# wengroup/matten

Hardware: NVIDIA B200
Metric: crystals/sec (inference fwd) (higher is better)
Workload: dtype f32

## Files before the change

matten_b200/csrc/conv_fwd_tc.cu:

```cuda
#include <stdlib.h>

#include <cub/device/device_scan.cuh>

#include "conv_fwd_tc.cuh"

namespace mt {

constexpr size_t kTcSmemLimit = (size_t)227 * 1024 - 1024;

static int tc_pick_ne(const mt_conv_tc_part& part, int y_lmax) {
  static const int cand[] = {256, 128, 80, 64, 48, 32};
  const int y_pad = sh_pad_len(y_lmax);
  for (int ne : cand) {
    if (2 * part.num_tiles * ne > 512) continue;
    const TcSmemLayout L = tc_smem_layout(part.a_rows, part.x_cols, y_pad, part.num_bi, ne);
    if (L.total <= kTcSmemLimit) return ne;
  }
  return 0;
}

static bool tc_plan_qualifies(const mt_conv_plan* plan) {
  if (plan->tc_num_parts <= 0 || plan->tc_num_parts > MT_TC_MAX_PARTS) return false;
  if (plan->tc_y_lmax < 0 || plan->tc_y_lmax > MT_LMAX) return false;
  if (plan->mlp_num_layers > 3) return false;
// ... 78 lines not shown
  const TcLayout L = tc_layout(y_lmax, N, E);
  MT_REQUIRE(layout && layout_bytes >= L.total && (reinterpret_cast<uintptr_t>(layout) & 255) == 0,
             "conv layout: buffer of mt_conv_layout_bytes() bytes, 256-byte aligned, required");
  MT_REQUIRE(rowptr && (E == 0 || (sh && perm && src_sorted)), "null pointer");
  return tc_prepare_layout(L, reinterpret_cast<uintptr_t>(layout), y_lmax, static_cast<const float*>(sh), rowptr, perm,
                           src_sorted, N, as_stream(stream));
}

size_t conv_fwd_tc_workspace_bytes(const mt_conv_plan* plan, int64_t N, int64_t E) {
  if (!tc_plan_qualifies(plan) || N <= 0) return 0;
  return tc_workspace_bytes(tc_layout(plan->tc_y_lmax, N, E));
}

static long long* g_tc_dbg = nullptr;
void conv_fwd_tc_set_debug(void* p) { g_tc_dbg = static_cast<long long*>(p); }

typedef CUresult (*EncodeTiledFn)(CUtensorMap*, CUtensorMapDataType, cuuint32_t, void*, const cuuint64_t*, const cuuint64_t*,
                                  const cuuint32_t*, const cuuint32_t*, CUtensorMapInterleave, CUtensorMapSwizzle,
                                  CUtensorMapL2promotion, CUtensorMapFloatOOBfill);

static EncodeTiledFn encode_tiled_fn() {
  static EncodeTiledFn fn = nullptr;
  static bool tried = false;
  if (!tried) {
    void* p = nullptr;
    cudaDriverEntryPointQueryResult q;
    if (cudaGetDriverEntryPoint("cuTensorMapEncodeTiled", &p, cudaEnableDefault, &q) == cudaSuccess &&
        q == cudaDriverEntryPointSuccess)
      fn = reinterpret_cast<EncodeTiledFn>(p);
    tried = true;
  }
  return fn;
}

int conv_fwd_tc_try(const mt_conv_plan* plan, const void* x, const void* sh, const void* emb,
                    const void* const* mlp_weights, const int32_t* rowptr, const int32_t* perm,
                    const int32_t* src_sorted, double avg, const void* num_neigh, void* out, void* workspace,
                    size_t workspace_bytes, const void* layout, int64_t N, int64_t E, cudaStream_t st, int* used) {
  *used = 0;
  if (!tc_plan_qualifies(plan)) return MT_OK;
  if (E + 3 * N >= (int64_t)2147483647 || N >= (int64_t)2147483647) return MT_OK;
  const TcLayout L = tc_layout(plan->tc_y_lmax, N, E);
  if (workspace == nullptr || workspace_bytes < tc_workspace_bytes(L)) return MT_OK;
  if ((reinterpret_cast<uintptr_t>(x) & 15) != 0) return MT_OK;
  EncodeTiledFn encode = encode_tiled_fn();
  if (encode == nullptr) return set_error(MT_ECUDA, "cuTensorMapEncodeTiled is not available from this driver");
  ConvTcParams p;
  memset(&p, 0, sizeof(p));
  p.x_dim = plan->x_dim;
  p.y_dim = plan->y_dim;
  p.y_lmax = plan->tc_y_lmax;
  p.out_dim = plan->out_dim;
  p.nl = plan->mlp_num_layers;
  for (int i = 0; i <= p.nl; ++i) p.sizes[i] = plan->mlp_sizes[i];
  for (int i = 0; i < p.nl; ++i) p.w[i] = static_cast<const float*>(mlp_weights[i]);
  p.act = plan->mlp_act;
  p.act_cst = (float)plan->mlp_act_cst;
  p.emb = static_cast<const float*>(emb);
  p.rowptr = rowptr;
  p.perm = perm;
  p.src = src_sorted;
  p.avg = (float)avg;
  p.num_neigh = static_cast<const float*>(num_neigh);
  p.out = static_cast<float*>(out);
  p.N = N;
  p.E = E;
  p.num_parts = plan->tc_num_parts;
  p.dbg = g_tc_dbg;
  {
    const uintptr_t base = (reinterpret_cast<uintptr_t>(workspace) + 255) & ~(uintptr_t)255;
    if (layout == nullptr) {
      const int rc = tc_prepare_layout(L, base, plan->tc_y_lmax, static_cast<const float*>(sh), rowptr, perm, src_sorted,
                                       N, st);
      if (rc != MT_OK) return rc;
      layout = reinterpret_cast<const void*>(base);
    }
    const uintptr_t lb = reinterpret_cast<uintptr_t>(layout);
    p.rowptr_pad = reinterpret_cast<int32_t*>(lb + L.rowptr_pad) + (N + 1);
    p.orig_pad = reinterpret_cast<int32_t*>(lb + L.orig_pad);
    p.src_pad = reinterpret_cast<int32_t*>(lb + L.src_pad);
    p.ypairs = reinterpret_cast<float*>(lb + L.ypairs);
    p.hplanes = reinterpret_cast<__nv_bfloat16*>(base + L.total);
    p.cols_max = L.cols_max;
    const bool fast = p.nl == 3 && p.sizes[0] <= 8 && p.sizes[1] == kTcK && p.sizes[2] == kTcK && p.act == MT_ACT_SILU;
    int64_t g = ceil_div<int64_t>(L.cols_max, fast ? 256 : 64);
    if (g > (int64_t)kNumSMs * 8) g = (int64_t)kNumSMs * 8;
    if (g < 1) g = 1;
    if (fast) tc_edge_hidden_fast_kernel<<<(unsigned)g, 256, 0, st>>>(p);
    else tc_edge_hidden_kernel<<<(unsigned)g, kHidThreads, 0, st>>>(p);
    MT_LAUNCH_OK();
  }
  int64_t grid = kNumSMs;
  if (grid > N * p.num_parts) grid = N * p.num_parts;
  if (grid < p.num_parts) grid = p.num_parts;
  double cost_sum = 0;
  for (int i = 0; i < p.num_parts; ++i) cost_sum += plan->tc_parts[i].cost > 0 ? plan->tc_parts[i].cost : 1;
  int assigned = 0;
  int lmax = 0;
  TcMaps maps;
  memset(&maps, 0, sizeof(maps));
  size_t smem_max = 0;
  for (int i = 0; i < p.num_parts; ++i) {
    const mt_conv_tc_part& pt = plan->tc_parts[i];
    TcPartParams& q = p.part[i];
    q.num_tiles = pt.num_tiles;
    q.a_rows = pt.a_rows;
    q.num_bi = pt.num_bi;
    q.x_lo = pt.x_lo;
    q.x_cols = pt.x_cols;
    q.ne = tc_pick_ne(pt, plan->tc_y_lmax);
    for (int k = 0; k < 4; ++k) q.q_count[k] = pt.q_count[k];
    q.row_wcol = pt.row_wcol;
    q.bi_hdr = pt.bi_hdr;
    q.bi_lane = pt.bi_lane;
    q.q_list = pt.q_list;
    const double c = pt.cost > 0 ? pt.cost : 1;
    int n = (i + 1 == p.num_parts) ? (int)grid - assigned : (int)((double)grid * c / cost_sum + 0.5);
    const int left = p.num_parts - 1 - i;
    if (n > (int)grid - assigned - left) n = (int)grid - assigned - left;
    if (n < 1) n = 1;
    if (n > N && N > 0) n = (int)N;
    q.cta_first = assigned;
    q.cta_count = n;
    assigned += n;
    if (pt.lmax > lmax) lmax = pt.lmax;
    const TcSmemLayout L = tc_smem_layout(q.a_rows, q.x_cols, sh_pad_len(p.y_lmax), q.num_bi, q.ne);
    if (L.total > smem_max) smem_max = L.total;
    cuuint64_t dims[2] = {(cuuint64_t)plan->x_dim, (cuuint64_t)(N > 0 ? N : 1)};
    cuuint64_t strides[1] = {(cuuint64_t)plan->x_dim * 4};
    cuuint32_t box[2] = {(cuuint32_t)q.x_cols, 1};
    cuuint32_t estr[2] = {1, 1};
    const CUresult r = encode(&maps.m[i], CU_TENSOR_MAP_DATA_TYPE_FLOAT32, 2, const_cast<void*>(x), dims, strides, box, estr,
                              CU_TENSOR_MAP_INTERLEAVE_NONE, CU_TENSOR_MAP_SWIZZLE_NONE, CU_TENSOR_MAP_L2_PROMOTION_NONE,
                              CU_TENSOR_MAP_FLOAT_OOB_FILL_NONE);
    if (r != CUDA_SUCCESS) return set_error(MT_ECUDA, "cuTensorMapEncodeTiled failed (%d)", (int)r);
    cuuint64_t hdims[3] = {16, (cuuint64_t)p.cols_max, 12};
    cuuint64_t hstrides[2] = {16, (cuuint64_t)p.cols_max * 16};
    cuuint32_t hbox[3] = {16, (cuuint32_t)q.ne, 12};
    cuuint32_t hestr[3] = {1, 1, 1};
    const CUresult rh = encode(&maps.h[i], CU_TENSOR_MAP_DATA_TYPE_UINT8, 3, p.hplanes, hdims, hstrides, hbox, hestr,
                               CU_TENSOR_MAP_INTERLEAVE_NONE, CU_TENSOR_MAP_SWIZZLE_NONE, CU_TENSOR_MAP_L2_PROMOTION_NONE,
                               CU_TENSOR_MAP_FLOAT_OOB_FILL_NONE);
    if (rh != CUDA_SUCCESS) return set_error(MT_ECUDA, "cuTensorMapEncodeTiled (h planes) failed (%d)", (int)rh);
  }
  grid = assigned;
  static thread_local size_t configured[2] = {0, 0};
  const int vi = lmax <= 2 ? 0 : 1;
  if (smem_max > configured[vi]) {
    if (vi == 0)
      MT_CUDA_OK(cudaFuncSetAttribute(conv_fwd_tc_kernel<2>, cudaFuncAttributeMaxDynamicSharedMemorySize, (int)kTcSmemLimit));
    else
      MT_CUDA_OK(cudaFuncSetAttribute(conv_fwd_tc_kernel<4>, cudaFuncAttributeMaxDynamicSharedMemorySize, (int)kTcSmemLimit));
    configured[vi] = kTcSmemLimit;
  }
  if (vi == 0) conv_fwd_tc_kernel<2><<<(unsigned)grid, kTcThreads, smem_max, st>>>(p, maps);
  else conv_fwd_tc_kernel<4><<<(unsigned)grid, kTcThreads, smem_max, st>>>(p, maps);
  MT_LAUNCH_OK();
  *used = 1;
  return MT_OK;
}

}
```

matten_b200/csrc/conv_fwd_tc.cuh:

```cuda
#pragma once
#include <cuda.h>
#include <cuda_bf16.h>

#include "common.cuh"
#include "generated/cg_bundles.cuh"

namespace mt {

constexpr int kTcK = 32;
constexpr int kTcProducerWarps = 4;
constexpr int kTcConsumerWarps = 16;
constexpr int kTcThreads = 32 * (kTcProducerWarps + kTcConsumerWarps);
constexpr int kTcMaxTiles = 4;
constexpr int kTcMaxBI = 64;
constexpr int kTcMaxNodes = 32;
constexpr int kTcMaxParts = 4;

__host__ __device__ constexpr int tc_chunk_cols(int MT) { return MT <= 1 ? 256 : (MT == 2 ? 128 : (MT == 3 ? 80 : 64)); }

struct TcPartParams {
  int num_tiles;
  int a_rows;
  int num_bi;
  int x_lo, x_cols;
// ... 81 lines not shown
}
__device__ __forceinline__ void fence_barrier_init() { asm volatile("fence.mbarrier_init.release.cluster;" ::: "memory"); }
__device__ __forceinline__ void fence_proxy_async() { asm volatile("fence.proxy.async.shared::cta;" ::: "memory"); }
__device__ __forceinline__ void tc_fence_before() { asm volatile("tcgen05.fence::before_thread_sync;" ::: "memory"); }
__device__ __forceinline__ void tc_fence_after() { asm volatile("tcgen05.fence::after_thread_sync;" ::: "memory"); }
__device__ __forceinline__ void tmem_alloc(uint32_t* dst_smem, uint32_t ncols) {
  asm volatile("tcgen05.alloc.cta_group::1.sync.aligned.shared::cta.b32 [%0], %1;" ::"r"(smem_u32(dst_smem)), "r"(ncols)
               : "memory");
  asm volatile("tcgen05.relinquish_alloc_permit.cta_group::1.sync.aligned;" ::: "memory");
}
__device__ __forceinline__ void tmem_dealloc(uint32_t taddr, uint32_t ncols) {
  asm volatile("tcgen05.dealloc.cta_group::1.sync.aligned.b32 %0, %1;" ::"r"(taddr), "r"(ncols) : "memory");
}
__device__ __forceinline__ void umma_commit(uint64_t* bar) {
  asm volatile("tcgen05.commit.cta_group::1.mbarrier::arrive::one.shared::cluster.b64 [%0];" ::"r"(smem_u32(bar))
               : "memory");
}
__device__ __forceinline__ void umma_bf16(uint32_t d_tmem, uint64_t a_desc, uint64_t b_desc, uint32_t idesc,
                                          uint32_t accumulate) {
  asm volatile(
      "{\n"
      ".reg .pred p;\n"
      "setp.ne.b32 p, %4, 0;\n"
      "tcgen05.mma.cta_group::1.kind::f16 [%0], %1, %2, %3, p;\n"
      "}\n" ::"r"(d_tmem),
      "l"(a_desc), "l"(b_desc), "r"(idesc), "r"(accumulate)
      : "memory");
}
struct W4 {
  uint32_t a, b, c, d;
};
__device__ __forceinline__ void tmem_ld_x4(uint32_t taddr, W4& r) {
  asm volatile("tcgen05.ld.sync.aligned.32x32b.x4.b32 {%0, %1, %2, %3}, [%4];"
               : "=r"(r.a), "=r"(r.b), "=r"(r.c), "=r"(r.d)
               : "r"(taddr));
}
__device__ __forceinline__ void tmem_ld_16x256b(uint32_t taddr, W4& r) {
  asm volatile("tcgen05.ld.sync.aligned.16x256b.x1.b32 {%0, %1, %2, %3}, [%4];"
               : "=r"(r.a), "=r"(r.b), "=r"(r.c), "=r"(r.d)
               : "r"(taddr));
}
__device__ __forceinline__ void tmem_ld_wait(W4& r) {
  asm volatile("tcgen05.wait::ld.sync.aligned;" : "+r"(r.a), "+r"(r.b), "+r"(r.c), "+r"(r.d));
}
__device__ __forceinline__ void tmem_ld_touch(W4& r) {
  asm volatile("" : "+r"(r.a), "+r"(r.b), "+r"(r.c), "+r"(r.d));
}

__device__ __forceinline__ void tma_gather4(void* dst_smem, const CUtensorMap* map, int col, int r0, int r1, int r2, int r3,
                                            uint64_t* bar) {
  asm volatile(
      "cp.async.bulk.tensor.2d.shared::cta.global.tile::gather4.mbarrier::complete_tx::bytes.cta_group::1 "
      "[%0], [%1, {%2, %3, %4, %5, %6}], [%7];" ::"r"(smem_u32(dst_smem)),
      "l"(map), "r"(col), "r"(r0), "r"(r1), "r"(r2), "r"(r3), "r"(smem_u32(bar))
      : "memory");
}

__device__ __forceinline__ void tma_load_3d(void* dst_smem, const CUtensorMap* map, int c0, int c1, int c2, uint64_t* bar) {
  asm volatile(
      "cp.async.bulk.tensor.3d.shared::cluster.global.tile.mbarrier::complete_tx::bytes [%0], [%1, {%2, %3, %4}], [%5];" ::"r"(
          smem_u32(dst_smem)),
      "l"(map), "r"(c0), "r"(c1), "r"(c2), "r"(smem_u32(bar))
      : "memory");
}

__device__ __forceinline__ void bulk_g2s(void* dst_smem, const void* src_gmem, uint32_t bytes, uint64_t* bar) {
  asm volatile("cp.async.bulk.shared::cluster.global.mbarrier::complete_tx::bytes [%0], [%1], %2, [%3];" ::"r"(
                   smem_u32(dst_smem)),
               "l"(src_gmem), "r"(bytes), "r"(smem_u32(bar))
               : "memory");
}

__device__ __forceinline__ uint64_t make_kmajor_desc(uint32_t start_addr, uint32_t lbo_bytes, uint32_t sbo_bytes) {
  uint64_t d = 0;
  d |= (uint64_t)((start_addr >> 4) & 0x3FFF);
  d |= (uint64_t)((lbo_bytes >> 4) & 0x3FFF) << 16;
  d |= (uint64_t)((sbo_bytes >> 4) & 0x3FFF) << 32;
  d |= (uint64_t)1 << 46;
  return d;
}
__device__ __forceinline__ constexpr uint32_t make_idesc_bf16(int M, int N) {
  return (1u << 4) | (1u << 7) | (1u << 10) | ((uint32_t)(N >> 3) << 17) | ((uint32_t)(M >> 4) << 24);
}

__device__ __forceinline__ void split_bf16x3(float v, __nv_bfloat16& hi, __nv_bfloat16& mi, __nv_bfloat16& lo) {
  hi = __float2bfloat16_rn(v);
  const float r1 = v - __bfloat162float(hi);
  mi = __float2bfloat16_rn(r1);
  const float r2 = r1 - __bfloat162float(mi);
  lo = __float2bfloat16_rn(r2);
}

#define MT_TC_TIMER() const bool _tm = (p.dbg != nullptr) && blockIdx.x == 0; unsigned _tl = _tm ? (unsigned)clock() : 0u; unsigned _ta[8] = {0, 0, 0, 0, 0, 0, 0, 0}
#define MT_TACC(i) do { if (_tm) { const unsigned _n = (unsigned)clock(); _ta[i] += (_n - _tl) >> 4; _tl = _n; } } while (0)
#define MT_TC_TIMER_FLUSH() do { if (_tm && lane == 0) { for (int _i = 0; _i < 8; ++_i) p.dbg[warp * 8 + _i] = (long long)_ta[_i] << 4; } } while (0)

struct __align__(16) TcMeta {
  int nnodes;
  int ncols;
  int continues;
  int pc0;
  int node_id[kTcMaxNodes];
  float inv_den[kTcMaxNodes];
  short cb[kTcMaxNodes];
  short ngrp[kTcMaxNodes];
  unsigned char first[kTcMaxNodes];
};

struct TcSmemLayout {
  size_t a_off, a_plane;
  size_t b_off, b_plane;
  size_t x_off, x_buf;
  size_t y_off, y_buf;
  size_t meta_off;
  size_t lane_off;
  size_t hdr_off;
  size_t qlist_off;
  size_t total;
};
__host__ __device__ inline size_t tc_align(size_t v, size_t a = 128) { return (v + a - 1) & ~(a - 1); }
__host__ __device__ inline int tc_pad8(int v) { return (v + 7) & ~7; }
__host__ __device__ inline TcSmemLayout tc_smem_layout(int a_rows, int x_cols, int y_pad, int num_bi, int NE) {
  TcSmemLayout L;
  size_t o = 0;
  L.a_off = o;
  L.a_plane = (size_t)a_rows * kTcK * 2;
  o += 3 * L.a_plane;
  L.b_off = o;
  L.b_plane = (size_t)NE * kTcK * 2;
  o = tc_align(o + 3 * L.b_plane);
  L.x_off = o;
  L.x_buf = tc_align((size_t)NE * x_cols * 4);
  o += 2 * L.x_buf;
  L.y_off = o;
  L.y_buf = tc_align((size_t)(NE / 2) * 2 * y_pad * 4);
  o += 2 * L.y_buf;
  L.meta_off = o;
  o = tc_align(o + 2 * tc_align(sizeof(TcMeta), 16));
  L.lane_off = o;
  o += (size_t)num_bi * 32 * 16;
  L.hdr_off = o;
  o += (size_t)num_bi * 32;
  L.qlist_off = o;
  o = tc_align(o + 4 * kTcMaxBI);
  L.total = o;
  return L;
}

struct TcUnit {
  uint32_t tstage;
  int quarter;
  int ne;
  int slot[3];
  unsigned mask;
  int nch;
  const float* xs;
  int xstride;
  const float* ys;
  int ystride;
  int cb, ngrp;
  int4 lt;
  float* out;
  float inv_den;
  bool first;
};

// ... 153 lines not shown
      const W4& t = wsel[p >> 1];
      const float w0 = __uint_as_float((p & 1) ? t.c : t.a), w1 = __uint_as_float((p & 1) ? t.d : t.b);
      w2[p] = active ? f2(w0, w1) : f2(0.f, 0.f);
    }
    B::template edge<f2>(x2, y2, w2, acc, mask);
    __syncwarp();
  }
#pragma unroll
  for (int i = 0; i < B::NACC; ++i) {
    float s = acc[i].v.x + acc[i].v.y;
    s += __shfl_xor_sync(0xffffffffu, s, 1);
    s += __shfl_xor_sync(0xffffffffu, s, 2);
    for (int o = 4 << lg; o < 32; o <<= 1) s += __shfl_xor_sync(0xffffffffu, s, o);
    acc[i] = f2(s, 0.f);
  }
  tc_store<B>(acc, u, mask);
}

template <int ID>
__device__ __forceinline__ void tc_unit_dispatch(const TcUnit u, int mode, int lane) {
  using B = Bundle<ID>;
  const bool full = u.mask == (1u << B::NP) - 1u;
  if (mode == 0) {
    if (full) tc_unit_L<B, true>(u);
    else tc_unit_L<B, false>(u);
  } else {
    if (full) tc_unit_P<B, true>(u, lane);
    else tc_unit_P<B, false>(u, lane);
  }
}

__device__ __forceinline__ float tc_fast_sigmoid(float v) {
  float e, r;
  asm("ex2.approx.ftz.f32 %0, %1;" : "=f"(e) : "f"(-1.4426950408889634f * v));
  asm("rcp.approx.ftz.f32 %0, %1;" : "=f"(r) : "f"(1.0f + e));
  return r;
}
__device__ __forceinline__ void tc_split8(const float (&v)[8], uint4& hi, uint4& mi, uint4& lo) {
  uint32_t H[4], M[4], Lo[4];
#pragma unroll
  for (int i = 0; i < 4; ++i) {
    const float a = v[2 * i], b = v[2 * i + 1];
    const __nv_bfloat162 h2 = __floats2bfloat162_rn(a, b);
    const uint32_t hb = *reinterpret_cast<const uint32_t*>(&h2);
    const float ra = a - __uint_as_float(hb << 16), rb = b - __uint_as_float(hb & 0xffff0000u);
    const __nv_bfloat162 m2 = __floats2bfloat162_rn(ra, rb);
    const uint32_t mb = *reinterpret_cast<const uint32_t*>(&m2);
    const float sa = ra - __uint_as_float(mb << 16), sb = rb - __uint_as_float(mb & 0xffff0000u);
    const __nv_bfloat162 l2 = __floats2bfloat162_rn(sa, sb);
    H[i] = hb;
    M[i] = mb;
    Lo[i] = *reinterpret_cast<const uint32_t*>(&l2);
  }
  hi = make_uint4(H[0], H[1], H[2], H[3]);
  mi = make_uint4(M[0], M[1], M[2], M[3]);
  lo = make_uint4(Lo[0], Lo[1], Lo[2], Lo[3]);
}

__global__ void __launch_bounds__(256) tc_pad_degree_kernel(const int32_t* __restrict__ rowptr, int64_t N,
                                                            int32_t* __restrict__ degp) {
  const int64_t n = blockIdx.x * (int64_t)blockDim.x + threadIdx.x;
  if (n < N) degp[n] = (rowptr[n + 1] - rowptr[n] + 3) & ~3;
  if (n == N) degp[n] = 0;
}

__global__ void __launch_bounds__(256) tc_pad_layout_kernel(const int32_t* __restrict__ rowptr,
                                                            const int32_t* __restrict__ rowptr_pad,
                                                            const int32_t* __restrict__ perm, const int32_t* __restrict__ src,
                                                            int64_t N, int32_t* __restrict__ orig_pad,
                                                            int32_t* __restrict__ src_pad) {
  const int lane = threadIdx.x & 31;
  for (int64_t n = (blockIdx.x * (int64_t)blockDim.x + threadIdx.x) >> 5; n < N; n += ((int64_t)gridDim.x * blockDim.x) >> 5) {
    const int r0 = rowptr[n], deg = rowptr[n + 1] - r0;
    const int c0 = rowptr_pad[n], degp = rowptr_pad[n + 1] - c0;
    for (int t = lane; t < degp; t += 32) {
      const int e = r0 + (t < deg ? t : deg - 1);
      const int o = perm[e];
      orig_pad[c0 + t] = (t < deg) ? o : (-1 - o);
      src_pad[c0 + t] = src[e];
    }
  }
}

constexpr int kHidThreads = 256;
__global__ void __launch_bounds__(kHidThreads) tc_edge_hidden_kernel(const ConvTcParams p) {
  __shared__ __align__(16) float sW[2 * kTcK * kTcK];
  __shared__ float sV[(kHidThreads / 32) * 8 * 33];
  const int nh = p.nl - 1;
  for (int li = 0; li < nh; ++li) {
    const int fi = p.sizes[li], fo = p.sizes[li + 1];
    const float s = rsqrtf((float)fi);
    for (int t = threadIdx.x; t < kTcK * kTcK; t += kHidThreads) {
      const int k = t >> 5, j = t & 31;
      sW[li * kTcK * kTcK + t] = (k < fi && j < fo) ? p.w[li][(size_t)k * fo + j] * s : 0.f;
    }
  }
  __syncthreads();
  const int lane = threadIdx.x & 31, warp = threadIdx.x >> 5;
  const int q4 = lane & 3, cl = lane >> 2;
  const int in0 = p.sizes[0];
  float* vrow = sV + (warp * 8 + cl) * 33;
  const int64_t cols = p.rowptr_pad[p.N];
  uint4* planes = reinterpret_cast<uint4*>(p.hplanes);
  const int64_t wpb = kHidThreads / 32;
  for (int64_t c0 = (blockIdx.x * wpb + warp) * 8; c0 < cols; c0 += (int64_t)gridDim.x * wpb * 8) {
    const int64_t c = c0 + cl;
    const bool in = c < cols;
    const int oe = in ? p.orig_pad[c] : 0;
    const bool real = in && oe >= 0;
    const int64_t orig = oe >= 0 ? oe : (-1 - oe);
    const float* er = p.emb + orig * in0;
    __syncwarp();
#pragma unroll
    for (int i = 0; i < 8; ++i) {
      const int idx = 8 * q4 + i;
      vrow[idx] = (real && idx < in0) ? er[idx] : 0.f;
    }
    __syncwarp();
#pragma unroll 1
    for (int li = 0; li < nh; ++li) {
      const int K = p.sizes[li], fo = p.sizes[li + 1];
      const float* W = sW + li * kTcK * kTcK + 8 * q4;
      float2 a[4];
#pragma unroll
      for (int i = 0; i < 4; ++i) a[i] = make_float2(0.f, 0.f);
#pragma unroll 8
      for (int kk = 0; kk < K; ++kk) {
        const float hk = vrow[kk];
        const float4* wr = reinterpret_cast<const float4*>(W + kk * kTcK);
        const float4 w0 = wr[0], w1 = wr[1];
        fma_pair(hk, w0.x, w0.y, a[0]);
        fma_pair(hk, w0.z, w0.w, a[1]);
        fma_pair(hk, w1.x, w1.y, a[2]);
        fma_pair(hk, w1.z, w1.w, a[3]);
      }
      __syncwarp();
      float o8[8];
#pragma unroll
      for (int i = 0; i < 4; ++i) {
        o8[2 * i] = a[i].x;
        o8[2 * i + 1] = a[i].y;
      }
      if (p.act == MT_ACT_SILU) {
#pragma unroll
        for (int i = 0; i < 8; ++i) o8[i] = o8[i] * tc_fast_sigmoid(o8[i]);
      } else {
#pragma unroll 1
        for (int i = 0; i < 8; ++i) o8[i] = apply_act<float>(p.act, o8[i]);
      }
#pragma unroll
      for (int i = 0; i < 8; ++i) vrow[8 * q4 + i] = (8 * q4 + i < fo) ? o8[i] * p.act_cst : 0.f;
      __syncwarp();
    }
    if (in) {
      float h8[8];
#pragma unroll
      for (int i = 0; i < 8; ++i) h8[i] = real ? vrow[8 * q4 + i] : 0.f;
      uint4 hi, mi, lo;
      tc_split8(h8, hi, mi, lo);
      planes[(size_t)(0 * 4 + q4) * p.cols_max + c] = hi;
      planes[(size_t)(1 * 4 + q4) * p.cols_max + c] = mi;
      planes[(size_t)(2 * 4 + q4) * p.cols_max + c] = lo;
    }
  }
}

__global__ void __launch_bounds__(256) tc_ypairs_kernel(const float* __restrict__ sh, const int32_t* __restrict__ rowptr_pad,
                                                        const int32_t* __restrict__ orig_pad, int64_t N, int ylmax,
                                                        float* __restrict__ ypairs) {
  const int yn = (ylmax + 1) * (ylmax + 1);
  const int ystride = 2 * sh_pad_len(ylmax);
  const int64_t cols = rowptr_pad[N];
  for (int64_t c = blockIdx.x * 256ll + threadIdx.x; c < cols; c += (int64_t)gridDim.x * 256) {
    const int oe = orig_pad[c];
    const int64_t orig = oe >= 0 ? oe : (-1 - oe);
    const float* __restrict__ yr = sh + orig * yn;
    float* yo = ypairs + (c >> 1) * ystride + (c & 1);
#pragma unroll
    for (int l = 0; l <= MT_LMAX; ++l) {
      if (l <= ylmax) {
#pragma unroll
        for (int k = 0; k < 2 * l + 1; ++k) yo[2 * (sh_pad_pos(l) + k)] = yr[l * l + k];
      }
    }
  }
}

__global__ void __launch_bounds__(256, 3) tc_edge_hidden_fast_kernel(const ConvTcParams p) {
  __shared__ __align__(16) float sW0[8 * kTcK];
  __shared__ __align__(16) float sW1[kTcK * kTcK];
  const int in0 = p.sizes[0];
  {
    const float s0 = rsqrtf((float)in0), s1 = rsqrtf((float)kTcK);
    for (int t = threadIdx.x; t < 8 * kTcK; t += 256) sW0[t] = (t >> 5) < in0 ? p.w[0][t] * s0 : 0.f;
    for (int t = threadIdx.x; t < kTcK * kTcK; t += 256) sW1[t] = p.w[1][t] * s1;
  }
  __syncthreads();
  const uint32_t cols = p.rowptr_pad[p.N];
  uint4* planes = reinterpret_cast<uint4*>(p.hplanes);
  const float cst = p.act_cst;
  const bool emb_vec = in0 == 8 && (reinterpret_cast<uintptr_t>(p.emb) & 15) == 0;
  for (uint32_t c = blockIdx.x * 256 + threadIdx.x; c < cols; c += gridDim.x * 256) {
    const int oe = p.orig_pad[c];
    const bool real = oe >= 0;
    const int64_t orig = real ? oe : (-1 - oe);
    float h0[8];
    if (emb_vec) {
      const float4* er = reinterpret_cast<const float4*>(p.emb + orig * 8);
      const float4 a = er[0], b = er[1];
      h0[0] = a.x; h0[1] = a.y; h0[2] = a.z; h0[3] = a.w;
      h0[4] = b.x; h0[5] = b.y; h0[6] = b.z; h0[7] = b.w;
    } else {
      const float* er = p.emb + orig * in0;
#pragma unroll
      for (int i = 0; i < 8; ++i) h0[i] = i < in0 ? er[i] : 0.f;
    }
    float2 acc[16];
    float h1[kTcK];
#pragma unroll
    for (int i = 0; i < 16; ++i) acc[i] = make_float2(0.f, 0.f);
#pragma unroll
    for (int k = 0; k < 8; ++k) {
      const float4* wr = reinterpret_cast<const float4*>(sW0 + k * kTcK);
#pragma unroll
      for (int j = 0; j < 8; ++j) {
        const float4 w = wr[j];
        fma_pair(h0[k], w.x, w.y, acc[2 * j]);
        fma_pair(h0[k], w.z, w.w, acc[2 * j + 1]);
      }
    }
#pragma unroll
    for (int i = 0; i < 16; ++i) {
      h1[2 * i] = acc[i].x * tc_fast_sigmoid(acc[i].x) * cst;
      h1[2 * i + 1] = acc[i].y * tc_fast_sigmoid(acc[i].y) * cst;
      acc[i] = make_float2(0.f, 0.f);
    }
#pragma unroll
    for (int k = 0; k < kTcK; ++k) {
      const float4* wr = reinterpret_cast<const float4*>(sW1 + k * kTcK);
#pragma unroll
      for (int j = 0; j < 8; ++j) {
        const float4 w = wr[j];
        fma_pair(h1[k], w.x, w.y, acc[2 * j]);
        fma_pair(h1[k], w.z, w.w, acc[2 * j + 1]);
      }
    }
#pragma unroll
    for (int g = 0; g < 4; ++g) {
      float h8[8];
#pragma unroll
      for (int i = 0; i < 4; ++i) {
        const float a = acc[4 * g + i].x, b = acc[4 * g + i].y;
        h8[2 * i] = real ? a * tc_fast_sigmoid(a) * cst : 0.f;
        h8[2 * i + 1] = real ? b * tc_fast_sigmoid(b) * cst : 0.f;
      }
      uint4 hi, mi, lo;
      tc_split8(h8, hi, mi, lo);
      planes[(size_t)(0 * 4 + g) * p.cols_max + c] = hi;
      planes[(size_t)(1 * 4 + g) * p.cols_max + c] = mi;
      planes[(size_t)(2 * 4 + g) * p.cols_max + c] = lo;
    }
  }
}

template <int LMAXK>
__global__ void __launch_bounds__(kTcThreads, 1) conv_fwd_tc_kernel(const __grid_constant__ ConvTcParams p,
                                                                   const __grid_constant__ TcMaps maps) {
  extern __shared__ __align__(128) unsigned char smem[];
  __shared__ uint64_t bar_full[2], bar_empty[2], bar_go[2], bar_bready, bar_bfree;
  __shared__ uint32_t s_tmem_base;
  __shared__ int s_cnt[2][4];
  __shared__ int s_mma_b;

  const int tid = threadIdx.x, lane = tid & 31, warp = tid >> 5;
  int part_id = 0;
#pragma unroll
  for (int i = 1; i < kTcMaxParts; ++i)
    if (i < p.num_parts && (int)blockIdx.x >= p.part[i].cta_first) part_id = i;
  const TcPartParams& P = p.part[part_id];
  const int MT = P.num_tiles, NE = P.ne, a_rows = P.a_rows;
  const int y_pad = sh_pad_len(p.y_lmax);
  const int ystride = 2 * y_pad;
  const TcSmemLayout L = tc_smem_layout(a_rows, P.x_cols, y_pad, P.num_bi, NE);
  unsigned char* sA = smem + L.a_off;
  unsigned char* sB = smem + L.b_off;
  unsigned char* sMeta = smem + L.meta_off;
  constexpr size_t kMetaBytes = (sizeof(TcMeta) + 15) & ~(size_t)15;
  int4* sLane = reinterpret_cast<int4*>(smem + L.lane_off);
  int* sHdr = reinterpret_cast<int*>(smem + L.hdr_off);
  unsigned char* sQ = smem + L.qlist_off;

  if (tid == 0) {
    mbar_init(&bar_full[0], 2);
    mbar_init(&bar_full[1], 2);
    mbar_init(&bar_empty[0], kTcConsumerWarps);
    mbar_init(&bar_empty[1], kTcConsumerWarps);
    mbar_init(&bar_go[0], 1);
    mbar_init(&bar_go[1], 1);
    mbar_init(&bar_bready, 1);
    mbar_init(&bar_bfree, 1);
    fence_barrier_init();
  }
  if (warp == 0) tmem_alloc(&s_tmem_base, 512);
  for (int t = tid; t < P.num_bi * 32; t += kTcThreads) sLane[t] = reinterpret_cast<const int4*>(P.bi_lane)[t];
  for (int t = tid; t < P.num_bi * 8; t += kTcThreads) sHdr[t] = P.bi_hdr[t];
  for (int t = tid; t < 4 * kTcMaxBI; t += kTcThreads) sQ[t] = (unsigned char)P.q_list[t];
  {
    uint4* z = reinterpret_cast<uint4*>(smem + L.b_off);
    const int n16 = (int)((L.meta_off - L.b_off) >> 4);
    for (int t = tid; t < n16; t += kTcThreads) z[t] = make_uint4(0u, 0u, 0u, 0u);
  }
  {
    const int H = p.sizes[p.nl - 1], Wn = p.sizes[p.nl];
    const float* __restrict__ Wl = p.w[p.nl - 1];
    const float s = rsqrtf((float)H);
    for (int t = tid; t < a_rows * 4; t += kTcThreads) {
      const int R = t >> 2, g = t & 3;
      const int wc = P.row_wcol[R];
      float v[8];
#pragma unroll
      for (int i = 0; i < 8; ++i) {
        const int k = g * 8 + i;
        v[i] = (wc >= 0 && k < H) ? Wl[(size_t)k * Wn + wc] * s : 0.f;
      }
      uint4 hi, mi, lo;
      tc_split8(v, hi, mi, lo);
      const size_t off = (size_t)g * a_rows * 16 + (size_t)R * 16;
      *reinterpret_cast<uint4*>(sA + off) = hi;
      *reinterpret_cast<uint4*>(sA + L.a_plane + off) = mi;
      *reinterpret_cast<uint4*>(sA + 2 * L.a_plane + off) = lo;
    }
  }
  fence_proxy_async();
  tc_fence_before();
  __syncthreads();
  tc_fence_after();
  const uint32_t tmem_base = s_tmem_base;

  if (warp == 0) {
    int64_t n_cur, n_end;
    {
      const int64_t rank = (int64_t)blockIdx.x - P.cta_first, cnt = P.cta_count;
      auto bound = [&](int64_t i) -> int64_t {
// ... 64 lines not shown
      int m = (fm == 0xffffffffu) ? 32 : (__ffs(~fm) - 1);
      const bool split0 = __shfl_sync(0xffffffffu, (int)split, 0) != 0;
      if (split0) m = 1;
      const bool mine = lane < m;
      const int cb = cum - degp;
      const float inv_den = mine ? (p.num_neigh ? rsqrtf(p.num_neigh[cand]) : rsqrtf(p.avg)) : 0.f;
      const int ncols = __shfl_sync(0xffffffffu, cum, m - 1);
      const int pc0 = __shfl_sync(0xffffffffu, c_lo, 0);
      MT_TACC(0);
      if (lane == 0) mbar_wait(&bar_empty[b], ((k >> 1) & 1) ^ 1, 10 + b);
      __syncwarp();
      MT_TACC(1);
      if (mine) {
        M.node_id[lane] = (int)cand;
        M.cb[lane] = (short)cb;
        M.ngrp[lane] = (short)(degp >> 2);
        M.first[lane] = (lane == 0 && c_carry >= 0) ? 0 : 1;
        M.inv_den[lane] = inv_den;
      }
      const bool continues = (c_carry >= 0);
      if (lane == 0) {
        M.nnodes = m;
        M.ncols = ncols;
        M.pc0 = pc0;
        s_cnt[b][0] = 0; s_cnt[b][1] = 0; s_cnt[b][2] = 0; s_cnt[b][3] = 0;
        if (continues && k > 0) mbar_wait(&bar_empty[b ^ 1], ((k - 1) >> 1) & 1, 12);
      }
      __syncwarp();
      if (ncols == 0) {
        if (lane == 0) {
          mbar_arrive(&bar_go[b]);
          mbar_arrive(&bar_full[b]);
          mbar_arrive(&bar_full[b]);
        }
      } else {
        if (lane == 0) {
          mbar_arrive_expect_tx(&bar_full[b], (uint32_t)ncols * xrow_bytes + (uint32_t)(ncols >> 1) * ypair_bytes);
          mbar_arrive(&bar_go[b]);
          if (b_uses > 0) mbar_wait(&bar_bfree, (b_uses - 1) & 1, 21);
          s_mma_b = b;
          mbar_arrive_expect_tx(&bar_bready, (uint32_t)NE * 16u * 12u);
        }
        __syncwarp();
        MT_TACC(2);
        if (lane == 0) {
          tma_load_3d(sB, &maps.h[part_id], 0, pc0, 0, &bar_bready);
        } else if (lane == 12) {
          bulk_g2s(smem + L.y_off + (size_t)b * L.y_buf, p.ypairs + (size_t)(pc0 >> 1) * ystride,
                   (uint32_t)(ncols >> 1) * ypair_bytes, &bar_full[b]);
        }
        ++b_uses;
        MT_TACC(3);
      }
      if (split0) {
        c_carry = pc0 + NE;
        if (c_carry >= __shfl_sync(0xffffffffu, c_hi, 0)) {
          c_carry = -1;
          n_cur += 1;
        }
      } else {
        c_carry = -1;
        n_cur += m;
      }
    }
    MT_TC_TIMER_FLUSH();
  } else if (warp == 1) {
    const uint32_t idesc = make_idesc_bf16(128, NE);
    const uint32_t a_lbo = (uint32_t)a_rows * 16, b_lbo = (uint32_t)NE * 16;
    const uint32_t a_plane32 = (uint32_t)L.a_plane, b_plane32 = (uint32_t)L.b_plane;
    const uint64_t a_desc0 = make_kmajor_desc(smem_u32(sA), a_lbo, 128);
    const uint64_t b_desc0 = make_kmajor_desc(smem_u32(sB), b_lbo, 128);
    MT_TC_TIMER();
    for (int k = 0;; ++k) {
      int b = 0;
      if (lane == 0) {
        mbar_wait(&bar_bready, k & 1, 30);
        b = s_mma_b;
      }
      b = __shfl_sync(0xffffffffu, b, 0);
      MT_TACC(0);
      if (b < 0) break;
      if (lane == 0) {
        tc_fence_after();
        constexpr uint32_t kPa = 0u | (2u << 2) | (1u << 4) | (0u << 6) | (1u << 8) | (0u << 10);
        constexpr uint32_t kPb = 2u | (0u << 2) | (1u << 4) | (1u << 6) | (0u << 8) | (0u << 10);
        for (int t = 0; t < MT; ++t) {
          const uint32_t d = tmem_base + (uint32_t)((b * MT + t) * NE);
          uint32_t accum = 0;
#pragma unroll
          for (int q = 0; q < 6; ++q) {
#pragma unroll
            for (int ks = 0; ks < 2; ++ks) {
              const uint32_t a_off = ((kPa >> (2 * q)) & 3u) * a_plane32 + (uint32_t)(2 * ks) * a_lbo + (uint32_t)t * 128 * 16;
              const uint32_t b_off = ((kPb >> (2 * q)) & 3u) * b_plane32 + (uint32_t)(2 * ks) * b_lbo;
              umma_bf16(d, a_desc0 + (uint64_t)(a_off >> 4), b_desc0 + (uint64_t)(b_off >> 4), idesc, accum);
              accum = 1;
            }
          }
        }
        umma_commit(&bar_full[b]);
        umma_commit(&bar_bfree);
      }
      __syncwarp();
      MT_TACC(1);
    }
    MT_TC_TIMER_FLUSH();
  } else if (warp == 2 || warp == 3) {
    const int ngw = MT == 1 ? 2 : 1;
    const int gw = warp == 2 ? 0 : 1;
    if (gw < ngw) {
    const CUtensorMap* map = &maps.m[part_id];
    const uint32_t xrow_bytes = (uint32_t)P.x_cols * 4;
    MT_TC_TIMER();
    for (int k = 0;; ++k) {
      const int b = k & 1;
      const TcMeta& M = *reinterpret_cast<const TcMeta*>(sMeta + b * kMetaBytes);
      if (lane == 0) mbar_wait(&bar_go[b], (k >> 1) & 1, 50 + b);
      __syncwarp();
      MT_TACC(0);
      const int nn = M.nnodes, ncols = M.ncols, pc0 = M.pc0;
      if (nn < 0) break;
      unsigned char* xs = smem + L.x_off + (size_t)b * L.x_buf;
      for (int g = ngw * lane + gw; g < (ncols >> 2); g += 32 * ngw) {
        const int4 r = *reinterpret_cast<const int4*>(p.src_pad + pc0 + 4 * g);
        tma_gather4(xs + (size_t)(4 * g) * xrow_bytes, map, P.x_lo, r.x, r.y, r.z, r.w, &bar_full[b]);
      }
      MT_TACC(1);
    }
    MT_TC_TIMER_FLUSH();
    }
  } else {
    const int q = warp & 3;
    const int nbiq = P.q_count[q];
    MT_TC_TIMER();
    for (int k = 0;; ++k) {
      const int b = k & 1;
      if (lane == 0) mbar_wait(&bar_full[b], (k >> 1) & 1, 40 + b);
      __syncwarp();
      MT_TACC(0);
      tc_fence_after();
      const TcMeta& M = *reinterpret_cast<const TcMeta*>(sMeta + b * kMetaBytes);
      const int nn = M.nnodes;
      if (nn < 0) break;
      TcUnit u;
      u.tstage = tmem_base + (uint32_t)(b * MT * NE);
      u.quarter = q;
      u.ne = NE;
      u.xs = reinterpret_cast<const float*>(smem + L.x_off + (size_t)b * L.x_buf);
      u.xstride = P.x_cols;
      u.ys = reinterpret_cast<const float*>(smem + L.y_off + (size_t)b * L.y_buf);
      u.ystride = ystride;
      const int num_units = nbiq * nn;
      while (true) {
        int unit = 0;
        if (lane == 0) unit = atomicAdd(&s_cnt[b][q], 1);
        unit = __shfl_sync(0xffffffffu, unit, 0);
        if (unit >= num_units) break;
        const int si = unit / nn, nj = unit - si * nn;
        const int bi = sQ[q * kTcMaxBI + si];
        const int4 h0 = *reinterpret_cast<const int4*>(sHdr + bi * 8);
        const int4 h1 = *reinterpret_cast<const int4*>(sHdr + bi * 8 + 4);
        u.mask = (unsigned)h0.w;
        u.nch = h0.z;
        u.slot[0] = h1.y; u.slot[1] = h1.z; u.slot[2] = h1.w;
        u.lt = sLane[bi * 32 + lane];
        u.cb = M.cb[nj];
        u.ngrp = M.ngrp[nj];
        u.out = p.out + (size_t)M.node_id[nj] * p.out_dim;
        u.inv_den = M.inv_den[nj];
        u.first = M.first[nj] != 0;
        __syncwarp();
        switch (h0.x) {
#define MT_TC_CASE(ID) \
  case ID:             \
    tc_unit_dispatch<ID>(u, h0.y, lane); \
    break;
          MT_FOR_EACH_BUNDLE_L2(MT_TC_CASE)
// ... 30 lines not shown
```

Measured before the change: 137,900.

## Run edge radial MLP on tcgen05 tensor cores with bf16x3 split

Replaces the scalar-FMA edge hidden MLP kernels (generic and fast paths) with one templated kernel. It stages 128 edge columns per CTA as bf16 hi/mid/lo planes in shared memory and runs each layer as six UMMA passes into TMEM, then applies the activation after tcgen05.ld. For 8-wide inputs it prefetches the next tile's embeddings. The cost it targets is the FP32 FMA work of the small MLP. In exchange it adds a CTA-wide barrier and an mbarrier wait per layer, plus TMEM allocation that limits CTAs per SM, which may serialise a kernel that is small to begin with.

```diff
diff --git a/matten_b200/csrc/conv_fwd_tc.cu b/matten_b200/csrc/conv_fwd_tc.cu
--- a/matten_b200/csrc/conv_fwd_tc.cu
+++ b/matten_b200/csrc/conv_fwd_tc.cu
@@ -184,12 +184,10 @@
     p.ypairs = reinterpret_cast<float*>(lb + L.ypairs);
     p.hplanes = reinterpret_cast<__nv_bfloat16*>(base + L.total);
     p.cols_max = L.cols_max;
-    const bool fast = p.nl == 3 && p.sizes[0] <= 8 && p.sizes[1] == kTcK && p.sizes[2] == kTcK && p.act == MT_ACT_SILU;
-    int64_t g = ceil_div<int64_t>(L.cols_max, fast ? 256 : 64);
-    if (g > (int64_t)kNumSMs * 8) g = (int64_t)kNumSMs * 8;
-    if (g < 1) g = 1;
-    if (fast) tc_edge_hidden_fast_kernel<<<(unsigned)g, 256, 0, st>>>(p);
-    else tc_edge_hidden_kernel<<<(unsigned)g, kHidThreads, 0, st>>>(p);
+    int64_t g = ceil_div<int64_t>(L.cols_max, kHidCols);
+    if (g > (int64_t)kNumSMs * kHidCtasPerSM) g = (int64_t)kNumSMs * kHidCtasPerSM;
+    if (p.sizes[0] <= 8) tc_edge_hidden_kernel<8><<<(unsigned)g, kHidThreads, 0, st>>>(p);
+    else tc_edge_hidden_kernel<32><<<(unsigned)g, kHidThreads, 0, st>>>(p);
     MT_LAUNCH_OK();
   }
   int64_t grid = kNumSMs;
diff --git a/matten_b200/csrc/conv_fwd_tc.cuh b/matten_b200/csrc/conv_fwd_tc.cuh
--- a/matten_b200/csrc/conv_fwd_tc.cuh
+++ b/matten_b200/csrc/conv_fwd_tc.cuh
@@ -187,6 +187,9 @@
 __device__ __forceinline__ constexpr uint32_t make_idesc_bf16(int M, int N) {
   return (1u << 4) | (1u << 7) | (1u << 10) | ((uint32_t)(N >> 3) << 17) | ((uint32_t)(M >> 4) << 24);
 }
+
+constexpr uint32_t kPlanesA = 0u | (2u << 2) | (1u << 4) | (0u << 6) | (1u << 8) | (0u << 10);
+constexpr uint32_t kPlanesB = 2u | (0u << 2) | (1u << 4) | (1u << 6) | (0u << 8) | (0u << 10);
 
 __device__ __forceinline__ void split_bf16x3(float v, __nv_bfloat16& hi, __nv_bfloat16& mi, __nv_bfloat16& lo) {
   hi = __float2bfloat16_rn(v);
@@ -506,87 +509,197 @@
   }
 }
 
-constexpr int kHidThreads = 256;
-__global__ void __launch_bounds__(kHidThreads) tc_edge_hidden_kernel(const ConvTcParams p) {
-  __shared__ __align__(16) float sW[2 * kTcK * kTcK];
-  __shared__ float sV[(kHidThreads / 32) * 8 * 33];
+constexpr int kHidCols = 128;
+constexpr int kHidThreads = 2 * kHidCols;
+constexpr int kHidCtasPerSM = 4;
+constexpr uint32_t kHidAPlane = 4 * kHidCols * 16;
+constexpr uint32_t kHidBPlane = 4 * kTcK * 16;
+
+struct W8 {
+  uint32_t a, b, c, d, e, f, g, h;
+};
+__device__ __forceinline__ void tmem_ld_x8(uint32_t taddr, W8& r) {
+  asm volatile("tcgen05.ld.sync.aligned.32x32b.x8.b32 {%0, %1, %2, %3, %4, %5, %6, %7}, [%8];"
+               : "=r"(r.a), "=r"(r.b), "=r"(r.c), "=r"(r.d), "=r"(r.e), "=r"(r.f), "=r"(r.g), "=r"(r.h)
+               : "r"(taddr));
+}
+__device__ __forceinline__ void tmem_ld_wait8(W8& r) {
+  asm volatile("tcgen05.wait::ld.sync.aligned;"
+               : "+r"(r.a), "+r"(r.b), "+r"(r.c), "+r"(r.d), "+r"(r.e), "+r"(r.f), "+r"(r.g), "+r"(r.h));
+}
+__device__ __forceinline__ void tmem_ld_touch8(W8& r) {
+  asm volatile("" : "+r"(r.a), "+r"(r.b), "+r"(r.c), "+r"(r.d), "+r"(r.e), "+r"(r.f), "+r"(r.g), "+r"(r.h));
+}
+
+__device__ __noinline__ float tc_hid_act_generic(int act, float v) { return apply_act<float>(act, v); }
+
+__device__ __forceinline__ void tc_hid_put(unsigned char* planes, uint32_t plane_bytes, uint32_t off, const float (&v)[8]) {
+  uint4 hi, mi, lo;
+  tc_split8(v, hi, mi, lo);
+  *reinterpret_cast<uint4*>(planes + off) = hi;
+  *reinterpret_cast<uint4*>(planes + plane_bytes + off) = mi;
+  *reinterpret_cast<uint4*>(planes + 2 * plane_bytes + off) = lo;
+}
+
+__device__ __forceinline__ void tc_hid_store(const ConvTcParams& p, uint32_t c, int g, const float (&v)[8]) {
+  uint4* planes = reinterpret_cast<uint4*>(p.hplanes);
+  uint4 hi, mi, lo;
+  tc_split8(v, hi, mi, lo);
+  planes[(size_t)(0 * 4 + g) * p.cols_max + c] = hi;
+  planes[(size_t)(1 * 4 + g) * p.cols_max + c] = mi;
+  planes[(size_t)(2 * 4 + g) * p.cols_max + c] = lo;
+}
+
+template <int KIN>
+__device__ __forceinline__ void tc_hid_load(const ConvTcParams& p, uint32_t c, uint32_t cols, bool vec, int half,
+                                            float (&e)[16], bool& real) {
+  const int oe = c < cols ? p.orig_pad[c] : -1;
+  real = oe >= 0;
+#pragma unroll
+  for (int i = 0; i < 16; ++i) e[i] = 0.f;
+  if (!real || (KIN == 8 && half != 0)) return;
+  const int in0 = p.sizes[0];
+  const float* er = p.emb + (int64_t)oe * in0;
+  if (KIN == 8 && vec) {
+    const float4 a = reinterpret_cast<const float4*>(er)[0], b = reinterpret_cast<const float4*>(er)[1];
+    e[0] = a.x; e[1] = a.y; e[2] = a.z; e[3] = a.w;
+    e[4] = b.x; e[5] = b.y; e[6] = b.z; e[7] = b.w;
+  } else {
+#pragma unroll
+    for (int i = 0; i < (KIN == 8 ? 8 : 16); ++i)
+      if (16 * half + i < in0) e[i] = er[16 * half + i];
+  }
+}
+
+__device__ __forceinline__ void tc_hid_w8(const W8& r, float (&v)[8]) {
+  v[0] = __uint_as_float(r.a); v[1] = __uint_as_float(r.b); v[2] = __uint_as_float(r.c); v[3] = __uint_as_float(r.d);
+  v[4] = __uint_as_float(r.e); v[5] = __uint_as_float(r.f); v[6] = __uint_as_float(r.g); v[7] = __uint_as_float(r.h);
+}
+
+template <int KIN>
+__global__ void __launch_bounds__(kHidThreads, kHidCtasPerSM) tc_edge_hidden_kernel(const ConvTcParams p) {
+  __shared__ __align__(128) unsigned char sA[3 * kHidAPlane];
+  __shared__ __align__(128) unsigned char sB[2][3 * kHidBPlane];
+  __shared__ uint64_t bar;
+  __shared__ uint32_t s_tmem;
+  const int tid = threadIdx.x, warp = tid >> 5, m = tid & (kHidCols - 1), half = tid / kHidCols;
   const int nh = p.nl - 1;
-  for (int li = 0; li < nh; ++li) {
-    const int fi = p.sizes[li], fo = p.sizes[li + 1];
-    const float s = rsqrtf((float)fi);
-    for (int t = threadIdx.x; t < kTcK * kTcK; t += kHidThreads) {
-      const int k = t >> 5, j = t & 31;
-      sW[li * kTcK * kTcK + t] = (k < fi && j < fo) ? p.w[li][(size_t)k * fo + j] * s : 0.f;
-    }
-  }
+  if (tid < 4 * kTcK) {
+    for (int li = 0; li < nh; ++li) {
+      const int fi = p.sizes[li], fo = p.sizes[li + 1], j = tid & 31, g = tid >> 5;
+      const float s = rsqrtf((float)fi);
+      float v[8];
+#pragma unroll
+      for (int i = 0; i < 8; ++i) {
+        const int k = 8 * g + i;
+        v[i] = (k < fi && j < fo) ? p.w[li][(size_t)k * fo + j] * s : 0.f;
+      }
+      tc_hid_put(sB[li], kHidBPlane, (uint32_t)(g * kTcK + j) * 16, v);
+    }
+  }
+  if (tid == 0) {
+    mbar_init(&bar, 1);
+    fence_barrier_init();
+  }
+  if (warp == 0) tmem_alloc(&s_tmem, 32);
+  fence_proxy_async();
+  tc_fence_before();
   __syncthreads();
-  const int lane = threadIdx.x & 31, warp = threadIdx.x >> 5;
-  const int q4 = lane & 3, cl = lane >> 2;
-  const int in0 = p.sizes[0];
-  float* vrow = sV + (warp * 8 + cl) * 33;
-  const int64_t cols = p.rowptr_pad[p.N];
-  uint4* planes = reinterpret_cast<uint4*>(p.hplanes);
-  const int64_t wpb = kHidThreads / 32;
-  for (int64_t c0 = (blockIdx.x * wpb + warp) * 8; c0 < cols; c0 += (int64_t)gridDim.x * wpb * 8) {
-    const int64_t c = c0 + cl;
-    const bool in = c < cols;
-    const int oe = in ? p.orig_pad[c] : 0;
-    const bool real = in && oe >= 0;
-    const int64_t orig = oe >= 0 ? oe : (-1 - oe);
-    const float* er = p.emb + orig * in0;
-    __syncwarp();
-#pragma unroll
-    for (int i = 0; i < 8; ++i) {
-      const int idx = 8 * q4 + i;
-      vrow[idx] = (real && idx < in0) ? er[idx] : 0.f;
-    }
-    __syncwarp();
+  tc_fence_after();
+  const uint32_t tmem = s_tmem;
+  const uint32_t tmem_thr = tmem + ((uint32_t)(32 * (warp & 3)) << 16) + (uint32_t)(16 * half);
+  const uint32_t cols = p.rowptr_pad[p.N];
+  const uint32_t stride = gridDim.x * kHidCols;
+  const bool vec = p.sizes[0] == 8 && (reinterpret_cast<uintptr_t>(p.emb) & 15) == 0;
+  const int act = p.act;
+  const float cst = p.act_cst;
+  const uint32_t idesc = make_idesc_bf16(kHidCols, kTcK);
+  const uint64_t a_desc = make_kmajor_desc(smem_u32(sA), kHidCols * 16, 128);
+  const int kg0 = p.sizes[0] <= 16 ? 2 : 4;
+  uint32_t phase = 0;
+  float e[16];
+  bool real;
+  constexpr bool kAhead = KIN == 8;
+  uint32_t c = blockIdx.x * kHidCols + m;
+  if (kAhead) tc_hid_load<KIN>(p, c, cols, vec, half, e, real);
+  for (; c - m < cols; c += stride) {
+    if (!kAhead) tc_hid_load<KIN>(p, c, cols, vec, half, e, real);
+    const bool creal = real;
+#pragma unroll
+    for (int gg = 0; gg < 2; ++gg) {
+      const int g = 2 * half + gg;
+      float v[8];
+#pragma unroll
+      for (int i = 0; i < 8; ++i) v[i] = e[8 * gg + i];
+      if (nh == 0) {
+        if (c < cols) tc_hid_store(p, c, g, v);
+      } else if (g < kg0) {
+        tc_hid_put(sA, kHidAPlane, (uint32_t)(g * kHidCols + m) * 16, v);
+      }
+    }
+    if (kAhead) tc_hid_load<KIN>(p, c + stride, cols, vec, half, e, real);
+    for (int li = 0; li < nh; ++li) {
+      fence_proxy_async();
+      tc_fence_before();
+      __syncthreads();
+      tc_fence_after();
+      if (tid == 0) {
+        const uint64_t b_desc = make_kmajor_desc(smem_u32(sB[li]), kTcK * 16, 128);
+        const int ksteps = p.sizes[li] <= 16 ? 1 : 2;
+        uint32_t accum = 0;
 #pragma unroll 1
-    for (int li = 0; li < nh; ++li) {
-      const int K = p.sizes[li], fo = p.sizes[li + 1];
-      const float* W = sW + li * kTcK * kTcK + 8 * q4;
-      float2 a[4];
-#pragma unroll
-      for (int i = 0; i < 4; ++i) a[i] = make_float2(0.f, 0.f);
-#pragma unroll 8
-      for (int kk = 0; kk < K; ++kk) {
-        const float hk = vrow[kk];
-        const float4* wr = reinterpret_cast<const float4*>(W + kk * kTcK);
-        const float4 w0 = wr[0], w1 = wr[1];
-        fma_pair(hk, w0.x, w0.y, a[0]);
-        fma_pair(hk, w0.z, w0.w, a[1]);
-        fma_pair(hk, w1.x, w1.y, a[2]);
-        fma_pair(hk, w1.z, w1.w, a[3]);
-      }
+        for (int q = 0; q < 6; ++q) {
+          for (int ks = 0; ks < ksteps; ++ks) {
+            const uint32_t a_off = ((kPlanesA >> (2 * q)) & 3u) * kHidAPlane + (uint32_t)ks * 2 * kHidCols * 16;
+            const uint32_t b_off = ((kPlanesB >> (2 * q)) & 3u) * kHidBPlane + (uint32_t)ks * 2 * kTcK * 16;
+            umma_bf16(tmem, a_desc + (uint64_t)(a_off >> 4), b_desc + (uint64_t)(b_off >> 4), idesc, accum);
+            accum = 1;
+          }
+        }
+        umma_commit(&bar);
+      }
+      if ((tid & 31) == 0) mbar_wait(&bar, phase, 60);
       __syncwarp();
-      float o8[8];
-#pragma unroll
-      for (int i = 0; i < 4; ++i) {
-        o8[2 * i] = a[i].x;
-        o8[2 * i + 1] = a[i].y;
-      }
-      if (p.act == MT_ACT_SILU) {
-#pragma unroll
-        for (int i = 0; i < 8; ++i) o8[i] = o8[i] * tc_fast_sigmoid(o8[i]);
-      } else {
-#pragma unroll 1
-        for (int i = 0; i < 8; ++i) o8[i] = apply_act<float>(p.act, o8[i]);
-      }
-#pragma unroll
-      for (int i = 0; i < 8; ++i) vrow[8 * q4 + i] = (8 * q4 + i < fo) ? o8[i] * p.act_cst : 0.f;
-      __syncwarp();
-    }
-    if (in) {
-      float h8[8];
-#pragma unroll
-      for (int i = 0; i < 8; ++i) h8[i] = real ? vrow[8 * q4 + i] : 0.f;
-      uint4 hi, mi, lo;
-      tc_split8(h8, hi, mi, lo);
-      planes[(size_t)(0 * 4 + q4) * p.cols_max + c] = hi;
-      planes[(size_t)(1 * 4 + q4) * p.cols_max + c] = mi;
-      planes[(size_t)(2 * 4 + q4) * p.cols_max + c] = lo;
-    }
-  }
+      phase ^= 1;
+      tc_fence_after();
+      W8 r[2];
+      tmem_ld_x8(tmem_thr, r[0]);
+      tmem_ld_x8(tmem_thr + 8, r[1]);
+      tmem_ld_wait8(r[0]);
+      tmem_ld_touch8(r[1]);
+      const int fo = p.sizes[li + 1];
+      const bool last = li + 1 == nh;
+#pragma unroll
+      for (int gg = 0; gg < 2; ++gg) {
+        const int g = 2 * half + gg;
+        float v[8];
+        tc_hid_w8(r[gg], v);
+        if (act == MT_ACT_SILU) {
+#pragma unroll
+          for (int i = 0; i < 8; ++i) v[i] = v[i] * tc_fast_sigmoid(v[i]) * cst;
+        } else {
+#pragma unroll
+          for (int i = 0; i < 8; ++i) v[i] = tc_hid_act_generic(act, v[i]) * cst;
+        }
+        if (fo < kTcK) {
+#pragma unroll
+          for (int i = 0; i < 8; ++i) v[i] = 8 * g + i < fo ? v[i] : 0.f;
+        }
+        if (!last) {
+          tc_hid_put(sA, kHidAPlane, (uint32_t)(g * kHidCols + m) * 16, v);
+        } else if (c < cols) {
+          if (!creal) {
+#pragma unroll
+            for (int i = 0; i < 8; ++i) v[i] = 0.f;
+          }
+          tc_hid_store(p, c, g, v);
+        }
+      }
+    }
+  }
+  tc_fence_before();
+  __syncthreads();
+  if (warp == 0) tmem_dealloc(tmem, 32);
 }
 
 __global__ void __launch_bounds__(256) tc_ypairs_kernel(const float* __restrict__ sh, const int32_t* __restrict__ rowptr_pad,
@@ -606,83 +719,6 @@
 #pragma unroll
         for (int k = 0; k < 2 * l + 1; ++k) yo[2 * (sh_pad_pos(l) + k)] = yr[l * l + k];
       }
-    }
-  }
-}
-
-__global__ void __launch_bounds__(256, 3) tc_edge_hidden_fast_kernel(const ConvTcParams p) {
-  __shared__ __align__(16) float sW0[8 * kTcK];
-  __shared__ __align__(16) float sW1[kTcK * kTcK];
-  const int in0 = p.sizes[0];
-  {
-    const float s0 = rsqrtf((float)in0), s1 = rsqrtf((float)kTcK);
-    for (int t = threadIdx.x; t < 8 * kTcK; t += 256) sW0[t] = (t >> 5) < in0 ? p.w[0][t] * s0 : 0.f;
-    for (int t = threadIdx.x; t < kTcK * kTcK; t += 256) sW1[t] = p.w[1][t] * s1;
-  }
-  __syncthreads();
-  const uint32_t cols = p.rowptr_pad[p.N];
-  uint4* planes = reinterpret_cast<uint4*>(p.hplanes);
-  const float cst = p.act_cst;
-  const bool emb_vec = in0 == 8 && (reinterpret_cast<uintptr_t>(p.emb) & 15) == 0;
-  for (uint32_t c = blockIdx.x * 256 + threadIdx.x; c < cols; c += gridDim.x * 256) {
-    const int oe = p.orig_pad[c];
-    const bool real = oe >= 0;
-    const int64_t orig = real ? oe : (-1 - oe);
-    float h0[8];
-    if (emb_vec) {
-      const float4* er = reinterpret_cast<const float4*>(p.emb + orig * 8);
-      const float4 a = er[0], b = er[1];
-      h0[0] = a.x; h0[1] = a.y; h0[2] = a.z; h0[3] = a.w;
-      h0[4] = b.x; h0[5] = b.y; h0[6] = b.z; h0[7] = b.w;
-    } else {
-      const float* er = p.emb + orig * in0;
-#pragma unroll
-      for (int i = 0; i < 8; ++i) h0[i] = i < in0 ? er[i] : 0.f;
-    }
-    float2 acc[16];
-    float h1[kTcK];
-#pragma unroll
-    for (int i = 0; i < 16; ++i) acc[i] = make_float2(0.f, 0.f);
-#pragma unroll
-    for (int k = 0; k < 8; ++k) {
-      const float4* wr = reinterpret_cast<const float4*>(sW0 + k * kTcK);
-#pragma unroll
-      for (int j = 0; j < 8; ++j) {
-        const float4 w = wr[j];
-        fma_pair(h0[k], w.x, w.y, acc[2 * j]);
-        fma_pair(h0[k], w.z, w.w, acc[2 * j + 1]);
-      }
-    }
-#pragma unroll
-    for (int i = 0; i < 16; ++i) {
-      h1[2 * i] = acc[i].x * tc_fast_sigmoid(acc[i].x) * cst;
-      h1[2 * i + 1] = acc[i].y * tc_fast_sigmoid(acc[i].y) * cst;
-      acc[i] = make_float2(0.f, 0.f);
-    }
-#pragma unroll
-    for (int k = 0; k < kTcK; ++k) {
-      const float4* wr = reinterpret_cast<const float4*>(sW1 + k * kTcK);
-#pragma unroll
-      for (int j = 0; j < 8; ++j) {
-        const float4 w = wr[j];
-        fma_pair(h1[k], w.x, w.y, acc[2 * j]);
-        fma_pair(h1[k], w.z, w.w, acc[2 * j + 1]);
-      }
-    }
-#pragma unroll
-    for (int g = 0; g < 4; ++g) {
-      float h8[8];
-#pragma unroll
-      for (int i = 0; i < 4; ++i) {
-        const float a = acc[4 * g + i].x, b = acc[4 * g + i].y;
-        h8[2 * i] = real ? a * tc_fast_sigmoid(a) * cst : 0.f;
-        h8[2 * i + 1] = real ? b * tc_fast_sigmoid(b) * cst : 0.f;
-      }
-      uint4 hi, mi, lo;
-      tc_split8(h8, hi, mi, lo);
-      planes[(size_t)(0 * 4 + g) * p.cols_max + c] = hi;
-      planes[(size_t)(1 * 4 + g) * p.cols_max + c] = mi;
-      planes[(size_t)(2 * 4 + g) * p.cols_max + c] = lo;
     }
   }
 }
@@ -913,8 +949,6 @@
       if (b < 0) break;
       if (lane == 0) {
         tc_fence_after();
-        constexpr uint32_t kPa = 0u | (2u << 2) | (1u << 4) | (0u << 6) | (1u << 8) | (0u << 10);
-        constexpr uint32_t kPb = 2u | (0u << 2) | (1u << 4) | (1u << 6) | (0u << 8) | (0u << 10);
         for (int t = 0; t < MT; ++t) {
           const uint32_t d = tmem_base + (uint32_t)((b * MT + t) * NE);
           uint32_t accum = 0;
@@ -922,8 +956,8 @@
           for (int q = 0; q < 6; ++q) {
 #pragma unroll
             for (int ks = 0; ks < 2; ++ks) {
-              const uint32_t a_off = ((kPa >> (2 * q)) & 3u) * a_plane32 + (uint32_t)(2 * ks) * a_lbo + (uint32_t)t * 128 * 16;
-              const uint32_t b_off = ((kPb >> (2 * q)) & 3u) * b_plane32 + (uint32_t)(2 * ks) * b_lbo;
+              const uint32_t a_off = ((kPlanesA >> (2 * q)) & 3u) * a_plane32 + (uint32_t)(2 * ks) * a_lbo + (uint32_t)t * 128 * 16;
+              const uint32_t b_off = ((kPlanesB >> (2 * q)) & 3u) * b_plane32 + (uint32_t)(2 * ks) * b_lbo;
               umma_bf16(d, a_desc0 + (uint64_t)(a_off >> 4), b_desc0 + (uint64_t)(b_off >> 4), idesc, accum);
               accum = 1;
             }
```

New measurement: 139,100, median of 6. No clear change (+0.9%).
